# dan11003/tbv_slam_public

Hardware: AMD Instinct MI355X
Metric: radar scan registrations/sec (400x3360 polar) (higher is better)
Workload: dtype u8 filter / f32 search / f64 solve

## Files before the change

tbv_slam_public_amd/csrc/matcher.hip:

```cpp
#include <algorithm>
#include <cfloat>
#include <cmath>
#include <memory>

#include "common.hpp"
#include "fastmath.hpp"

namespace {

#ifdef CFEAR_REG_TIMING
__device__ long long g_reg_t[32];
__device__ unsigned long long g_reg_sum[4];
#define REG_T0() long long _t0 = __builtin_readcyclecounter()
#define REG_TACC(k) do { const long long _t1 = __builtin_readcyclecounter(); \
    if (threadIdx.x == 0 && blockIdx.x == 0) g_reg_t[k] += _t1 - _t0; _t0 = _t1; } while (0)
#else
#define REG_T0()
#define REG_TACC(k)
#endif

constexpr int kMaxScans = kRegMaxScans;
constexpr int kRegDeferred = 1000;

struct MatchCommon {
  cfear_reg_params par;
  double angle_outlier;
  char* scratch;
  size_t scratch_stride;
  size_t job_stride;
  int32_t pairs_cap;
  int32_t dense_fields;
  uint32_t lds_total;
  int32_t cost_only;
  int32_t n_samples;
  int32_t samples_per_axis;
  int32_t only_deferred;
  int32_t take_all;
  int32_t final_launch;
  uint32_t lds_regular;
  cfear_reg_result* results;
  double xy_half, yaw_half;
  const cfear_reg_result* prior;
};

int reg_dense_fields(int cost) { return cost == CFEAR_P2P ? 3 : (cost == CFEAR_P2L ? 5 : 6); }

__host__ __device__ inline size_t match_bytes_global(int pairs_cap) { return ((size_t)pairs_cap * 2 + 255) / 256 * 256; }
size_t reg_scratch_bytes(int pairs_cap) { return match_bytes_global(pairs_cap) + ((size_t)pairs_cap * 52 + 255) / 256 * 256; }

struct Aff2 { double l0, l1, l2, l3, t0, t1; };

__device__ __forceinline__ Aff2 aff_from_xyt(const double* p) {
  double s, c;
  sincos(p[2], &s, &c);
  return Aff2{c, -s, s, c, p[0], p[1]};
}
__device__ __forceinline__ Aff2 aff_mul(const Aff2& a, const Aff2& b) {
  Aff2 r;
  r.l0 = a.l0 * b.l0 + a.l1 * b.l2;
  r.l1 = a.l0 * b.l1 + a.l1 * b.l3;
  r.l2 = a.l2 * b.l0 + a.l3 * b.l2;
  r.l3 = a.l2 * b.l1 + a.l3 * b.l3;
  r.t0 = a.l0 * b.t0 + a.l1 * b.t1 + a.t0;
  r.t1 = a.l2 * b.t0 + a.l3 * b.t1 + a.t1;
  return r;
}
__device__ __forceinline__ Aff2 aff_inv(const Aff2& a) {
  const double det = a.l0 * a.l3 - a.l2 * a.l1;
  const double invdet = 1.0 / det;
  Aff2 r;
  r.l0 = a.l3 * invdet; r.l1 = -a.l1 * invdet; r.l2 = -a.l2 * invdet; r.l3 = a.l0 * invdet;
  r.t0 = -(r.l0 * a.t0 + r.l1 * a.t1);
  r.t1 = -(r.l2 * a.t0 + r.l3 * a.t1);
  return r;
}

__device__ __forceinline__ double similarity(double x, double y) { return 2 * fmin(x, y) / (x + y); }
__device__ __forceinline__ double get_weight(int opt, double N1, double N2, double sim_dir, double plan1, double plan2) {
  switch (opt) {
    case 0: return 1.0;
    case 1: return similarity(N1, N2);
    case 2: return sim_dir;
    case 3: return similarity(plan1, plan2);
    case 4: return similarity(N1, N2) + sim_dir + similarity(plan1, plan2);
  }
  return 1.0;
}

__device__ __forceinline__ void loss_eval(int loss, double a, double w, double s, double& rho0, double& rho1) {
  const double dmin = DBL_MIN;
  switch (loss) {
    case 1: {
      const double b = a * a;
      if (s > b) {
        const double q = rsqrt_newton(s);
        rho0 = 2.0 * a * (s * q) - b; rho1 = fmax(dmin, a * q);
      } else { rho0 = s; rho1 = 1.0; }
      break;
    }
    case 2: {
      const double b = a * a, c = 1.0 / b;
      const double sum = 1.0 + s * c, inv = 1.0 / sum;
      rho0 = b * log(sum); rho1 = fmax(dmin, inv);
      break;
    }
    case 3: {
      const double b = a * a, c = 1.0 / b;
      const double sum = 1.0 + s * c, tmp = sqrt(sum);
      rho0 = 2.0 * b * (tmp - 1.0); rho1 = fmax(dmin, 1.0 / tmp);
      break;
    }
    case 4: {
      const double sum = 1.0 + s, inv = 1.0 / sum;
      const double g0 = log(sum), g1 = fmax(dmin, inv);
      double f0, f1;
      if (g0 > 1.0) { const double r = sqrt(g0); f0 = 2.0 * r - 1.0; f1 = fmax(dmin, 1.0 / r); }
      else { f0 = g0; f1 = 1.0; }
      rho0 = f0; rho1 = f1 * g1;
      break;
    }
    case 5: {
      const double a2 = a * a;
      if (s <= a2) { const double value = 1.0 - s / a2, vs = value * value; rho0 = a2 / 3.0 * (1.0 - vs * value); rho1 = vs; }
      else { rho0 = a2 / 3.0; rho1 = 0.0; }
      break;
    }
    default: rho0 = s; rho1 = 1.0;
  }
  rho0 *= w; rho1 *= w;
}

enum {
  S_X = 0, S_XCOST = 3, S_CUR = 4 , S_SCALE = 13, S_DIAG = 16, S_XNORM = 19, S_GMAX = 20, S_RADIUS = 21,
  S_DEC = 22, S_MINCOST = 23, S_MODEL = 24, S_CAND = 25, S_COS = 28, S_SIN = 29, S_ITCOST = 30, S_ITREL = 31, S_INIT = 32,
  S_LASTREL = 33, S_FINAL = 34, S_INTS = 35 , S_OUTER = 39 , S_COUNT = 48
};
enum { SI_ITER = 0, SI_REUSE = 1, SI_INVALID = 2, SI_PUSHED = 3, SI_USABLE = 4, SI_DONE = 5, SI_ITSUCC = 6, SI_FLAG = 7 };
constexpr int kMaxNW = 16;
constexpr size_t kPartOff = 0;
constexpr size_t kIpartOff = kMaxNW * 10 * 8;
constexpr size_t kStateOff = kIpartOff + 2 * kMaxNW * 4;
constexpr size_t kFixedLds = kStateOff + S_COUNT * 8;
constexpr int kPtrs = 6;

struct MtFit {
  size_t off_smean, off_match, off_region;
  int region;
  int tables_all;
  int dense_cap;
  bool gmatch;
  bool resident;
  bool can;
  bool good;
};
__host__ __device__ inline MtFit mt_fit(size_t lds_total, int last, int sum_pad, int max_pad, int n_src, int fields, bool allow_gmatch) {
  MtFit m;
  size_t off = kFixedLds + (size_t)last * (12 * 8 + kPtrs * 8 + 16) + ((((size_t)last + 1) * 4 + 15) & ~(size_t)15);
  m.off_smean = off; off += (size_t)n_src * 16;
  const size_t n_pairs = (size_t)last * n_src;
  const size_t match_bytes = ((n_pairs + 7) & ~(size_t)7) * 2;
  const size_t need_one = (size_t)kScanGridStartPad * 2 + (size_t)max_pad * 10;
  m.off_match = off;
  m.gmatch = allow_gmatch && ((off + match_bytes + 15) & ~(size_t)15) + need_one > lds_total;
  if (!m.gmatch) off += match_bytes;
  off = (off + 15) & ~(size_t)15;
  m.off_region = off;
  m.tables_all = (int)((size_t)last * kScanGridStartPad * 2 + (size_t)sum_pad * 10);
  const size_t per = (size_t)fields * 8 + 2;
  m.can = sum_pad <= 65535 && n_src < 65536 && off + need_one <= lds_total && off + 4096 <= lds_total;
  m.region = m.can ? (int)(lds_total - off) : 0;
  const size_t dense_all = ((n_pairs + 3) & ~(size_t)3) * per;
// ... 211 lines not shown
  const double i1 = rcp_newton(d1);
  const double t21 = A[7] - l20 * A[3];
  const double l21 = t21 * i1;
  const double d2 = A[8] - l20 * A[6] - l21 * t21;
  if (!(d2 > 0.0)) return false;
  const double i2 = rcp_newton(d2);
  const double z0 = b[0];
  const double z1 = b[1] - l10 * z0;
  const double z2 = b[2] - l20 * z0 - l21 * z1;
  y[2] = z2 * i2;
  y[1] = z1 * i1 - l21 * y[2];
  y[0] = z0 * i0 - l10 * y[1] - l20 * y[2];
  return isfinite(y[0]) && isfinite(y[1]) && isfinite(y[2]);
}

template <bool PIN = false>
__device__ __forceinline__ void sincos_pose(const double a, double* s, double* c) {
  if (fabs(a) <= 1e5) sincos_reduced<PIN>(a, s, c);
  else sincos(a, s, c);
}

struct MtSizes {
  int n_src, sum_pad, max_pad;
  int koff_lane;
  float4 geo_lane;
  bool grids_ok;
};
__device__ __forceinline__ MtSizes mt_sizes(const RegJob& job, const int last) {
  const int lane = threadIdx.x & 63;
  int n = 0;
  float4 g = make_float4(0.f, 0.f, 0.f, 1.f);
  if (lane <= last) n = gload<int>(job.scans[lane].n_cells);
  if (lane < last) g = gload_f4(job.scans[lane].grid_geo);
  const int np = lane < last ? scan_grid_pad(n) : 0;
  const int incl = wave_incl_scan_i32(np);
  MtSizes z;
  z.koff_lane = incl - np;
  z.geo_lane = g;
  z.sum_pad = __builtin_amdgcn_readlane(incl, 63);
  z.max_pad = __builtin_amdgcn_readlane(wave_incl_scan_max_i32(np), 63);
  z.n_src = __builtin_amdgcn_readlane(n, last);
  z.grids_ok = __ballot(lane < last && g.w != 1.f) == 0ull;
  return z;
}

template <int NT>
__device__ void mt_stage_once(const RegJob& job, const MtLds& f, const MtSizes& z) {
  const int tid = threadIdx.x, last = job.n_scans - 1;
  if (tid < last) { f.koff[tid] = z.koff_lane; f.ggeo[tid] = z.geo_lane; }
  if (tid == last) f.koff[last] = z.sum_pad;
  if (tid >= 64 && tid < 64 + last) {
    const int i = tid - 64;
    const Aff2 T = aff_from_xyt(job.poses[i]);
    double* k = f.kf + i * 12;
    k[0] = T.l0; k[1] = T.l1; k[2] = T.l2; k[3] = T.l3; k[4] = T.t0; k[5] = T.t1;
    const ScanView& tv = job.scans[i];
    const void** tp = f.tptr + i * kPtrs;
    tp[0] = tv.mean; tp[1] = tv.normal; tp[2] = tv.nsamples; tp[3] = tv.scale; tp[4] = tv.cov; tp[5] = tv.grid;
  }
  const ScanView& src = job.scans[last];
  for (int s = tid; s < z.n_src; s += NT) f.smean[s] = gload_d2(src.mean + s);
  __syncthreads();
}

template <int NT>
__device__ __forceinline__ void mt_restage(const MtLds& f, int i0, int i1) {
  const int tid = threadIdx.x;
  const int k_lo = f.koff[i0], NP = f.koff[i1] - k_lo;
  constexpr int kCs = kScanGridStartPad / 8;
  constexpr int kKf = NT >= 256 ? 4 : 1, kPer = 2;
  const int xy0 = (i1 - i0) * kCs, ix0 = xy0 + NP / 2;
  uint4* out = (uint4*)f.tables;
  auto dst_of = [&](int i, int j, int rel, int np) {
    return j < kCs ? (i - i0) * kCs + j : (j < kCs + np / 2 ? xy0 + rel / 2 + (j - kCs) : ix0 + rel / 8 + (j - kCs - np / 2));
  };
  for (int ib = i0; ib < i1; ib += kKf) {
    g_u32x4 v[kKf][kPer];
    int dst[kKf][kPer];
    unsigned add[kKf];
#pragma unroll
    for (int q = 0; q < kKf; q++) {
      const int i = ib + q;
#pragma unroll
      for (int h = 0; h < kPer; h++) dst[q][h] = -1;
      add[q] = 0u;
      if (i < i1) {
        const char* blob = (const char*)f.tptr[i * kPtrs + 5];
        const int rel = f.koff[i] - k_lo, np = f.koff[i + 1] - f.koff[i], pieces = kCs + np / 2 + np / 8;
        add[q] = (unsigned)rel * 0x10001u;
#pragma unroll
        for (int h = 0; h < kPer; h++) {
          const int j = tid + h * NT;
          if (j < pieces) {
            v[q][h] = gload<g_u32x4>(blob + (size_t)j * 16);
            dst[q][h] = dst_of(i, j, rel, np);
          }
        }
      }
    }
#pragma unroll
    for (int q = 0; q < kKf; q++)
#pragma unroll
      for (int h = 0; h < kPer; h++)
        if (dst[q][h] >= 0) {
          const unsigned a = dst[q][h] < xy0 ? add[q] : 0u;
          out[dst[q][h]] = make_uint4(v[q][h].x + a, v[q][h].y + a, v[q][h].z + a, v[q][h].w + a);
        }
    for (int i = ib; i < min(ib + kKf, i1); i++) {
      const char* blob = (const char*)f.tptr[i * kPtrs + 5];
      const int rel = f.koff[i] - k_lo, np = f.koff[i + 1] - f.koff[i], pieces = kCs + np / 2 + np / 8;
      for (int j = tid + kPer * NT; j < pieces; j += NT) {
        const g_u32x4 t = gload<g_u32x4>(blob + (size_t)j * 16);
        out[dst_of(i, j, rel, np)] = make_uint4(t.x, t.y, t.z, t.w);
      }
    }
  }
  __syncthreads();
}

template <int NT, bool SLOTS, int COST = -1>
__device__ int mt_associate(const RegJob& job, const MatchCommon& cm, int itr, const MtLds& f, const double* xsrc, double* gl_dense,
                            Dense& dn, int* ipart, int& iphase, bool& staged, const Slots* sl = nullptr) {
  const int tid = threadIdx.x, wave = tid >> 6, lane = tid & 63;
  const int last = job.n_scans - 1;
  const int n_src = gload<int>(job.scans[last].n_cells);
  const int n_pairs = last * n_src;
  const double curr_radius = (itr == 1) ? 2 * cm.par.radius : cm.par.radius;
  const double r2 = curr_radius * curr_radius;
  const float rwin = (float)curr_radius + 1e-3f;
  constexpr int G = kScanGrid;
  constexpr bool GM = NT >= 512;
  auto cost_is = [&](const int v) { return COST >= 0 ? COST == v : cm.par.cost == v; };
  const unsigned magic = n_src ? 0xFFFFFFFFu / (unsigned)n_src : 0u;
  auto split = [&](const int p, int& i, int& s) {
    unsigned q = __umulhi((unsigned)p, magic);
    int r = p - (int)q * n_src;
    if (r >= n_src) { q++; r -= n_src; }
    i = (int)q; s = r;
  };
  REG_T0();
  {
    const int k0 = tid - (NT - 64);
    if (k0 >= 0 && k0 < last) {
      const double* k = f.kf + k0 * 12;
      const Aff2 Ttar{k[0], k[1], k[2], k[3], k[4], k[5]};
      double sn, cs;
      sincos_pose<true>(xsrc[2], &sn, &cs);
      const Aff2 Tst = aff_mul(aff_inv(Ttar), Aff2{cs, -sn, sn, cs, xsrc[0], xsrc[1]});
      double* o = f.kf + k0 * 12 + 6;
      o[0] = Tst.l0; o[1] = Tst.l1; o[2] = Tst.l2; o[3] = Tst.l3; o[4] = Tst.t0; o[5] = Tst.t1;
    }
  }
  int accepted = 0;
  int pend_p = -1, pend_i = 0, pend_best = -1;
  double2 pend_ns = make_double2(0.0, 0.0), pend_nt = make_double2(0.0, 0.0);
  auto gate_pending = [&]() {
    if (pend_p < 0) return;
    int m = -1;
    if (pend_best >= 0) {
      const double* T = f.kf + pend_i * 12 + 6;
      const double nsx = T[0] * pend_ns.x + T[1] * pend_ns.y, nsy = T[2] * pend_ns.x + T[3] * pend_ns.y;
      if (fmax(nsx * pend_nt.x + nsy * pend_nt.y, 0.0) > cm.angle_outlier) m = pend_best;
    }
    if (GM && f.gmatch) gstore<unsigned short>(f.gmatch + pend_p, (unsigned short)m);
    else f.match[pend_p] = (unsigned short)m;
    accepted += (m >= 0);
  };
  for (int i0 = 0; i0 < last;) {
    int i1 = i0, bytes = 0;
    if (f.resident) i1 = last;
    else
      while (i1 < last) {
        const int b = kScanGridStartPad * 2 + (f.koff[i1 + 1] - f.koff[i1]) * 10;
        if (bytes + b > f.region) break;
        bytes += b; i1++;
      }
    if (i1 == i0) return -1;
    if (i0 > 0) __syncthreads();
    if (!(f.resident && staged)) mt_restage<NT>(f, i0, i1);
    else __syncthreads();
    REG_TACC(0);
    const int NP = f.koff[i1] - f.koff[i0];
    const float2* txy = (const float2*)(f.tables + (size_t)(i1 - i0) * kScanGridStartPad);
    const unsigned short* tix = (const unsigned short*)(txy + NP);
    const int lo = i0 * n_src, hi = i1 * n_src;
    int p = lo + ((tid - lo) & (NT - 1));
    for (; p < hi; p += NT) {
      int i, s;
      split(p, i, s);
      const double* T = f.kf + i * 12 + 6;
      const double2 u = f.smean[s];
      const double px = T[0] * u.x + T[1] * u.y + T[4];
      const double py = T[2] * u.x + T[3] * u.y + T[5];
      const float qx = (float)px, qy = (float)py;
      const float4 gg = f.ggeo[i];
      const int cx0 = min(G - 1, max(0, (int)floorf((qx - rwin - gg.x) * gg.z))), cx1 = min(G - 1, max(0, (int)floorf((qx + rwin - gg.x) * gg.z)));
      const int cy0 = min(G - 1, max(0, (int)floorf((qy - rwin - gg.y) * gg.z))), cy1 = min(G - 1, max(0, (int)floorf((qy + rwin - gg.y) * gg.z)));
      unsigned long long bestkey = ~0ull;
      auto visit = [&](const float2 c, const unsigned id) {
        const float dx = __fsub_rn(qx, c.x), dy = __fsub_rn(qy, c.y);
        const float d = __fadd_rn(__fmul_rn(dx, dx), __fmul_rn(dy, dy));
        const unsigned long long key = ((unsigned long long)__float_as_uint(d) << 32) | id;
        bestkey = key < bestkey ? key : bestkey;
      };
      const unsigned short* cs = f.tables + (i - i0) * kScanGridStartPad;
      auto scan_run = [&](int qb, int qe) {
        for (int q = qb; q < qe; q += 2) {
          const int qn = min(q + 1, qe - 1);
          const float2 ca = txy[q], cb = txy[qn];
          const unsigned ia = tix[q], ib = tix[qn];
          visit(ca, ia); visit(cb, ib);
        }
      };
      {
        const int r1 = min(cy0 + 1, cy1), r2c = min(cy0 + 2, cy1);
        const int b0 = cs[cy0 * G + cx0], e0 = cs[cy0 * G + cx1 + 1];
        const int b1 = cs[r1 * G + cx0], e1 = cs[r1 * G + cx1 + 1];
        const int b2 = cs[r2c * G + cx0], e2 = cs[r2c * G + cx1 + 1];
        scan_run(b0, e0);
        if (cy1 > cy0) scan_run(b1, e1);
        if (cy1 > cy0 + 1) scan_run(b2, e2);
        for (int cy = cy0 + 3; cy <= cy1; cy++) scan_run((int)cs[cy * G + cx0], (int)cs[cy * G + cx1 + 1]);
      }
      const int best = bestkey == ~0ull ? -1 : (int)(unsigned)(bestkey & 0xFFFFFFFFu);
      const float bestd = __uint_as_float((unsigned)(bestkey >> 32));
      gate_pending();
      pend_p = p; pend_i = i;
      pend_best = (best >= 0 && (double)bestd < r2) ? best : -1;
      if (pend_best >= 0) {
        pend_ns = gload_d2(job.scans[last].normal + s);
        pend_nt = gload_d2((const double2*)f.tptr[i * kPtrs + 1] + best);
      }
    }
    gate_pending();
    pend_p = -1;
    REG_TACC(1);
    i0 = i1;
  }
  staged = true;
  if (GM && f.gmatch) __threadfence_block();
  int base = 0, total = 0;
  if (!SLOTS) {
    const int incl = wave_incl_scan_i32(accepted);
    base = incl - accepted;
    int* buf = ipart + iphase * kMaxNW;
    if (lane == 63) buf[wave] = incl;
    __syncthreads();
    for (int wv = 0; wv < wave; wv++) base += buf[wv];
    int tt = buf[0];
#pragma unroll
    for (int wv = 1; wv < NT / 64; wv++) tt += buf[wv];
    total = __builtin_amdgcn_readfirstlane(tt);
    iphase ^= 1;
    dn.p = f.dense; dn.cap = f.dense_cap; dn.sidx = (unsigned short*)(f.dense + (size_t)cm.dense_fields * f.dense_cap); dn.smean = f.smean;
    dn.gp = gl_dense; dn.gcap = (size_t)cm.pairs_cap; dn.gsidx = (int*)(gl_dense + (size_t)cm.dense_fields * cm.pairs_cap);
    dn.n = total;
  }
  const size_t cap = SLOTS ? 0 : (size_t)dn.cap, gcap = SLOTS ? 0 : dn.gcap;
  REG_TACC(2);
  {
    struct Gathered {
      int best, i, s, tns, sns;
      double2 nt, tm, ns;
      double tsc, ssc;
      double4 S;
    };
    const ScanView& srcv = job.scans[last];
    auto match_at = [&](int p) -> int {
      if (p >= n_pairs) return 0xFFFF;
      return (GM && f.gmatch) ? (int)gload<unsigned short>(f.gmatch + p) : (int)f.match[p];
    };
    auto gather = [&](int best, int i, int s) {
      Gathered g;
      g.best = best;
      if (g.best == 0xFFFF) g.best = -1;
      g.i = i; g.s = s;
      if (g.best >= 0) {
        const void* const* tp = f.tptr + i * kPtrs;
        g.nt = gload_d2((const double2*)tp[1] + g.best);
        g.tm = gload_d2((const double2*)tp[0] + g.best);
        g.tns = gload<int>((const int32_t*)tp[2] + g.best);
        g.tsc = gload<double>((const double*)tp[3] + g.best);
        g.ns = gload_d2(srcv.normal + s);
        g.sns = gload<int>(srcv.nsamples + s);
        g.ssc = gload<double>(srcv.scale + s);
        if (cost_is(CFEAR_P2D)) g.S = gload_d4((const double4*)tp[4] + g.best);
      }
      return g;
    };
    int c = base, i, s;
    split(tid, i, s);
    int m_next = GM ? match_at(tid + NT) : 0;
    Gathered cur = gather(match_at(tid), i, s);
    for (int p = tid; p < n_pairs; p += NT) {
      split(p + NT, i, s);
      int m_use;
      if (GM) { m_use = m_next; m_next = match_at(p + 2 * NT); }
      else m_use = match_at(p + NT);
      const Gathered nxt = gather(m_use, i, s);
      if (cur.best >= 0) {
        const double* K = f.kf + cur.i * 12;
        const double* T = K + 6;
        const double2 nt = cur.nt, tm = cur.tm, ns = cur.ns;
        const double nsx = T[0] * ns.x + T[1] * ns.y, nsy = T[2] * ns.x + T[3] * ns.y;
        const double direction_similarity = fmax(nsx * nt.x + nsy * nt.y, 0.0);
        const double w = get_weight(cm.par.weight_opt, (double)cur.sns, (double)cur.tns,
                                    direction_similarity, cur.ssc, cur.tsc);
        double e[6];
        e[0] = K[0] * tm.x + K[1] * tm.y + K[4];
        e[1] = K[2] * tm.x + K[3] * tm.y + K[5];
        e[2] = w; e[3] = 0.0; e[4] = 0.0; e[5] = 0.0;
        if (cost_is(CFEAR_P2D)) {
          const double4 S = cur.S;
          const double a00 = K[0] * S.x + K[1] * S.z, a01 = K[0] * S.y + K[1] * S.w;
          const double a10 = K[2] * S.x + K[3] * S.z, a11 = K[2] * S.y + K[3] * S.w;
          const double c00 = (cm.par.regularization + (a00 * K[0] + a01 * K[1])) * cm.par.cov_scale;
          const double c01 = (0.0 + (a00 * K[2] + a01 * K[3])) * cm.par.cov_scale;
          const double c10 = (0.0 + (a10 * K[0] + a11 * K[1])) * cm.par.cov_scale;
          const double c11 = (cm.par.regularization + (a10 * K[2] + a11 * K[3])) * cm.par.cov_scale;
          const double det = c00 * c11 - c10 * c01, invdet = 1.0 / det;
          const double i00 = c11 * invdet, i10 = -c10 * invdet, i11 = c00 * invdet;
          const double l00 = sqrt(i00), l10 = i10 / l00;
          e[3] = l00; e[4] = l10; e[5] = sqrt(i11 - l10 * l10);
        } else if (cost_is(CFEAR_P2L)) {
          e[3] = K[0] * nt.x + K[1] * nt.y;
          e[4] = K[2] * nt.x + K[3] * nt.y;
        }
        if (SLOTS) {
          const int pp = p;
          sl->tmx[pp] = e[0]; sl->tmy[pp] = e[1]; sl->w[pp] = e[2]; sl->a0[pp] = e[3]; sl->a1[pp] = e[4]; sl->a2[pp] = e[5];
          sl->tidx[pp] = cur.best;
        } else {
          const int nf = COST == CFEAR_P2P ? 3 : (COST == CFEAR_P2L ? 5 : (COST == CFEAR_P2D ? 6 : cm.dense_fields));
          if (c < (int)cap) {
            dn.sidx[c] = (unsigned short)cur.s;
#pragma unroll
            for (int k = 0; k < 6; k++) if (k < nf) dn.p[k * cap + c] = e[k];
          } else {
            const size_t g = (size_t)c - cap;
            gstore<int>(dn.gsidx + g, cur.s);
#pragma unroll
            for (int k = 0; k < 6; k++) if (k < nf) gstore<double>(dn.gp + k * gcap + g, e[k]);
          }
        }
        c++;
      } else if (SLOTS) {
        sl->w[p] = -1.0; sl->tidx[p] = -1;
      }
      cur = nxt;
    }
  }
  if (SLOTS) return accepted;
  if (total > (int)cap) __threadfence_block();
  __syncthreads();
  REG_TACC(3);
  return total;
}

template <int NT, int COST, int LOSS>
__device__ void eval_all(const MatchCommon& cm, const Dense& dn, const double x[3], double c, double s, double out[10], double* part) {
  double acc[10];
#pragma unroll
  for (int k = 0; k < 10; k++) acc[k] = 0.0;
  const size_t cap = (size_t)dn.cap, gcap = dn.gcap;
  REG_T0();
  const int n_lds = min(dn.n, (int)cap);
  for (int i = threadIdx.x; i < n_lds; i += NT) {
    double a0 = 0.0, a1 = 0.0, a2 = 0.0;
    const int si = (int)dn.sidx[i];
    const double tmx = dn.p[i], tmy = dn.p[cap + i], w = dn.p[2 * cap + i];
    if (COST != CFEAR_P2P) { a0 = dn.p[3 * cap + i]; a1 = dn.p[4 * cap + i]; }
    if (COST == CFEAR_P2D) a2 = dn.p[5 * cap + i];
    const double2 sm = dn.smean[si];
    eval_slot<COST, LOSS, true>(cm.par, sm.x, sm.y, tmx, tmy, a0, a1, a2, w, x[0], x[1], c, s, acc);
  }
  constexpr int kTailU = COST == CFEAR_P2P ? 4 : 2;
  const int n_tail = dn.n - n_lds;
  for (int g0 = threadIdx.x; g0 < n_tail; g0 += kTailU * NT) {
    int si[kTailU];
    double tmx[kTailU], tmy[kTailU], w[kTailU], a0[kTailU], a1[kTailU], a2[kTailU];
#pragma unroll
    for (int u = 0; u < kTailU; u++) {
      const size_t g = (size_t)min(g0 + u * NT, n_tail - 1);
      si[u] = gload<int>(dn.gsidx + g);
      tmx[u] = gload<double>(dn.gp + g); tmy[u] = gload<double>(dn.gp + gcap + g); w[u] = gload<double>(dn.gp + 2 * gcap + g);
      a0[u] = a1[u] = a2[u] = 0.0;
      if (COST != CFEAR_P2P) { a0[u] = gload<double>(dn.gp + 3 * gcap + g); a1[u] = gload<double>(dn.gp + 4 * gcap + g); }
      if (COST == CFEAR_P2D) a2[u] = gload<double>(dn.gp + 5 * gcap + g);
    }
#pragma unroll
    for (int u = 0; u < kTailU; u++)
      if (g0 + u * NT < n_tail) {
// ... 41 lines not shown
        const double c0 = st[S_CAND], c1 = st[S_CAND + 1], c2 = st[S_CAND + 2];
        x_norm = sqrt_newton(c0 * c0 + c1 * c1 + c2 * c2);
        if (l0) {
          st[S_X] = c0; st[S_X + 1] = c1; st[S_X + 2] = c2;
#pragma unroll
          for (int k = 1; k < 10; k++) st[S_CUR + k - 1] = cnd[k];
        }
        x_cost = cand_cost;
        gradient_max_norm = fmax(fabs(cnd[1]), fmax(fabs(cnd[2]), fabs(cnd[3])));
        it_cost = x_cost; it_success = true;
        const double q = 2.0 * it_rel - 1.0;
        radius = radius * rcp_newton(fmax(1.0 / 3.0, 1.0 - q * q * q));
        radius = fmin(max_radius, radius);
        decrease_factor = 2.0; reuse_diagonal = false;
      } else {
        it_cost = cand_cost; it_success = false;
        radius = radius / decrease_factor; decrease_factor *= 2.0; reuse_diagonal = true;
      }
    }
    mt_lds_order();
  }
  while (proceed) {
    n_pushed++;
    last_rel = it_rel;
    min_iter_cost = fmin(min_iter_cost, it_cost);
    if (iteration >= max_iter || (it_success && gradient_max_norm <= gradient_tolerance) || radius <= min_radius) {
      done = 1;
      break;
    }
    iteration++;
    it_cost = 0.0; it_rel = 0.0; it_success = false;
    const double scale[3] = {st[S_SCALE], st[S_SCALE + 1], st[S_SCALE + 2]};
    double gs[3], Hs[9];
    {
      const double* cur = st + S_CUR - 1;
      gs[0] = cur[1] * scale[0]; gs[1] = cur[2] * scale[1]; gs[2] = cur[3] * scale[2];
      Hs[0] = cur[4] * scale[0] * scale[0]; Hs[1] = cur[5] * scale[0] * scale[1]; Hs[2] = cur[6] * scale[0] * scale[2];
      Hs[3] = Hs[1]; Hs[4] = cur[7] * scale[1] * scale[1]; Hs[5] = cur[8] * scale[1] * scale[2];
      Hs[6] = Hs[2]; Hs[7] = Hs[5]; Hs[8] = cur[9] * scale[2] * scale[2];
    }
    double diagonal[3];
    if (!reuse_diagonal) {
      diagonal[0] = fmin(fmax(Hs[0], min_lm_diagonal), max_lm_diagonal);
      diagonal[1] = fmin(fmax(Hs[4], min_lm_diagonal), max_lm_diagonal);
      diagonal[2] = fmin(fmax(Hs[8], min_lm_diagonal), max_lm_diagonal);
      if (l0) { st[S_DIAG] = diagonal[0]; st[S_DIAG + 1] = diagonal[1]; st[S_DIAG + 2] = diagonal[2]; }
    } else {
      diagonal[0] = st[S_DIAG]; diagonal[1] = st[S_DIAG + 1]; diagonal[2] = st[S_DIAG + 2];
    }
    double A[9];
#pragma unroll
    for (int k = 0; k < 9; k++) A[k] = Hs[k];
    const double inv_radius = rcp_newton(radius);
#pragma unroll
    for (int k = 0; k < 3; k++) A[k * 3 + k] += diagonal[k] * inv_radius;
    double y[3], step[3] = {0, 0, 0};
    const bool solved = chol3_solve(A, gs, y);
    reuse_diagonal = true;
    bool step_is_valid = false;
    model_cost_change = 0.0;
    if (solved) {
      step[0] = -y[0]; step[1] = -y[1]; step[2] = -y[2];
      const double sg = step[0] * gs[0] + step[1] * gs[1] + step[2] * gs[2];
      const double hs0 = Hs[0] * step[0] + Hs[1] * step[1] + Hs[2] * step[2];
      const double hs1 = Hs[3] * step[0] + Hs[4] * step[1] + Hs[5] * step[2];
      const double hs2 = Hs[6] * step[0] + Hs[7] * step[1] + Hs[8] * step[2];
      model_cost_change = -sg - (step[0] * hs0 + step[1] * hs1 + step[2] * hs2) / 2.0;
      step_is_valid = model_cost_change > 0.0;
    }
    if (!step_is_valid) {
      if (++num_consecutive_invalid_steps >= 5) { usable = false; done = 1; break; }
      radius = radius / decrease_factor; decrease_factor *= 2.0; reuse_diagonal = true;
      it_cost = x_cost; it_success = false; it_rel = 0.0;
      mt_lds_order();
      continue;
    }
    num_consecutive_invalid_steps = 0;
    double sn, cs;
    const double c2 = st[S_X + 2] + step[2] * scale[2];
    sincos_pose<true>(c2, &sn, &cs);
    if (l0) {
      st[S_CAND] = st[S_X] + step[0] * scale[0]; st[S_CAND + 1] = st[S_X + 1] + step[1] * scale[1]; st[S_CAND + 2] = c2;
      st[S_COS] = cs; st[S_SIN] = sn;
    }
    break;
  }
  if (l0) {
    st[S_XCOST] = x_cost; st[S_XNORM] = x_norm; st[S_GMAX] = gradient_max_norm; st[S_RADIUS] = radius; st[S_DEC] = decrease_factor;
    st[S_MINCOST] = min_iter_cost; st[S_MODEL] = model_cost_change; st[S_ITCOST] = it_cost; st[S_ITREL] = it_rel;
    st[S_LASTREL] = last_rel;
    if (done) st[S_FINAL] = fmin(st[S_INIT], min_iter_cost);
    si[SI_ITER] = iteration; si[SI_REUSE] = reuse_diagonal; si[SI_INVALID] = num_consecutive_invalid_steps;
    si[SI_PUSHED] = n_pushed; si[SI_USABLE] = usable; si[SI_DONE] = done; si[SI_ITSUCC] = it_success;
  }
}

template <int NT, int COST, int LOSS>
__device__ void lm_solve(const MatchCommon& cm, const Dense& dn, const int max_iter, double* part, double* st, const bool eval_only) {
  const bool w0 = (threadIdx.x >> 6) == 0;
  int* si = (int*)(st + S_INTS);
  double cnd[10];
  {
    const double x[3] = {st[S_OUTER], st[S_OUTER + 1], st[S_OUTER + 2]};
    double s0, c0;
    sincos_pose<true>(x[2], &s0, &c0);
    eval_all<NT, COST, LOSS>(cm, dn, x, c0, s0, cnd, part);
    if (eval_only) {
      if (threadIdx.x == 0) st[S_XCOST] = cnd[0];
      return;
    }
    if (w0) {
      if ((threadIdx.x & 63) == 0) {
        st[S_X] = x[0]; st[S_X + 1] = x[1]; st[S_X + 2] = x[2]; st[S_XCOST] = cnd[0];
#pragma unroll
        for (int k = 1; k < 10; k++) st[S_CUR + k - 1] = cnd[k];
        st[S_SCALE] = 1.0 / (1.0 + sqrt(cnd[4]));
        st[S_SCALE + 1] = 1.0 / (1.0 + sqrt(cnd[7]));
        st[S_SCALE + 2] = 1.0 / (1.0 + sqrt(cnd[9]));
        st[S_DIAG] = 0.0; st[S_DIAG + 1] = 0.0; st[S_DIAG + 2] = 0.0;
        st[S_XNORM] = sqrt_newton(x[0] * x[0] + x[1] * x[1] + x[2] * x[2]);
        st[S_GMAX] = fmax(fabs(cnd[1]), fmax(fabs(cnd[2]), fabs(cnd[3])));
        st[S_RADIUS] = 1e4; st[S_DEC] = 2.0; st[S_MINCOST] = cnd[0]; st[S_MODEL] = 0.0; st[S_ITCOST] = cnd[0]; st[S_ITREL] = 0.0;
        st[S_CAND] = x[0]; st[S_CAND + 1] = x[1]; st[S_CAND + 2] = x[2];
        st[S_INIT] = cnd[0]; st[S_LASTREL] = 0.0; st[S_FINAL] = cnd[0];
        si[SI_ITER] = 0; si[SI_REUSE] = 0; si[SI_INVALID] = 0; si[SI_PUSHED] = 0; si[SI_USABLE] = 1; si[SI_DONE] = 0; si[SI_ITSUCC] = 1;
      }
      mt_lds_order();
      lm_round(st, cnd, false, max_iter);
    }
  }
  for (;;) {
    REG_T0();
    __syncthreads();
    REG_TACC(21);
    if (__builtin_amdgcn_readfirstlane(si[SI_DONE])) break;
    const double cand[3] = {st[S_CAND], st[S_CAND + 1], st[S_CAND + 2]};
    const double cs = st[S_COS], sn = st[S_SIN];
    eval_all<NT, COST, LOSS>(cm, dn, cand, cs, sn, cnd, part);
    REG_TACC(22);
    if (w0) { __builtin_amdgcn_s_setprio(3); lm_round(st, cnd, true, max_iter); __builtin_amdgcn_s_setprio(0); }
    REG_TACC(16);
  }
}

__device__ __forceinline__ void write_capacity(cfear_reg_result* r, const double x[3]) {
  r->pose[0] = x[0]; r->pose[1] = x[1]; r->pose[2] = x[2];
  r->score = 0; r->final_cost = 0; r->num_residuals = 0; r->outer_iters = 0; r->lm_iters = 0;
  r->status = CFEAR_ERR_CAPACITY; r->last_relative_decrease = 0; r->reserved = 0;
}

template <int NW, int COST, int LOSS, bool CO, bool WIDE = false>
__global__ __launch_bounds__(NW * 64, WIDE ? 2 : ((NW == 4 && LOSS < 0) ? 3 : 4)) void matcher_kernel(const RegJob* __restrict__ jobs, const MatchCommon cm) {
  constexpr int NT = NW * 64;
#ifdef CFEAR_REG_TIMING
  if (blockIdx.x == 0 && blockIdx.y == 0 && threadIdx.x == 0 && g_reg_sum[1]) {
    printf("matcher launch: %llu workgroups, mean %llu cycles, longest %llu\n", g_reg_sum[1], g_reg_sum[0] / g_reg_sum[1], g_reg_sum[2]);
    g_reg_sum[0] = g_reg_sum[1] = g_reg_sum[2] = 0;
  }
  const long long t_total0 = __builtin_readcyclecounter();
#endif
  REG_T0();
  extern __shared__ __attribute__((aligned(16))) uint8_t smem[];
  const uint32_t lds_eff = cm.lds_total - (NW >= 8 ? (uint32_t)kPartBigBytes : 0u);
  double* part = NW >= 8 ? (double*)(smem + lds_eff) : (double*)(smem + kPartOff);
  int* ipart = (int*)(smem + kIpartOff);
  double* st = (double*)(smem + kStateOff);
  const RegJob& job = *(const RegJob*)((const char*)jobs + (size_t)blockIdx.x * cm.job_stride);
  const int m_out = CO ? (cm.n_samples > 0 ? cm.n_samples : 1) : 1;
  cfear_reg_result* res = cm.results + (size_t)blockIdx.x * m_out;
  if (cm.only_deferred && res->status != kRegDeferred) return;
  const int last = job.n_scans - 1;
  const MtSizes sz = mt_sizes(job, last);
  const int n_src = sz.n_src, sum_pad = sz.sum_pad, max_pad = sz.max_pad;
  const int n_pairs = last * n_src;
  const size_t scr_idx = (size_t)blockIdx.x * gridDim.y + blockIdx.y;
  char* scr = cm.scratch + scr_idx * cm.scratch_stride;
  const MtFit fit = mt_fit(lds_eff, last, sum_pad, max_pad, n_src, cm.dense_fields, NW >= 8);
  MtLds fl;
  const bool ok = fit.can && sz.grids_ok && n_pairs <= cm.pairs_cap && (cm.take_all || fit.good);
  REG_TACC(8);
  if (ok) {
    mt_carve(smem, fit, last, (unsigned short*)scr, fl);
    mt_stage_once<NT>(job, fl, sz);
  }
  REG_TACC(9);
  if (!ok) {
    if (cm.final_launch) {
      const double larger = (mt_fit((uint32_t)(160 * 1024 - 256 - kPartBigBytes), last, sum_pad, max_pad, n_src, cm.dense_fields, true).can &&
                             sz.grids_ok && n_pairs <= cm.pairs_cap && lds_eff < 160u * 1024u - 256u - (uint32_t)kPartBigBytes) ? 1.0 : 0.0;
      for (int sidx = blockIdx.y * NT + (int)threadIdx.x; sidx < m_out; sidx += (int)gridDim.y * NT) {
        write_capacity(res + sidx, job.poses[last]);
        res[sidx].reserved = larger;
      }
    } else if (threadIdx.x == 0) { res->status = kRegDeferred; res->reserved = 0.0; }
    return;
  }
  double* gl_dense = (double*)(scr + match_bytes_global(cm.pairs_cap));
  Dense dn;
  int iphase = 0;
  bool staged = false;
  const int rpb = COST == CFEAR_P2L ? 1 : 2;
  int git = job.itr ? job.itr : cm.par.itr;
  const bool from_prior = CO && cm.prior;
  if (from_prior) git = cm.prior[blockIdx.x].outer_iters;
  git = __builtin_amdgcn_readfirstlane(git);
  if (threadIdx.x == 0) {
    const double* x0 = from_prior ? cm.prior[blockIdx.x].pose : job.poses[last];
#pragma unroll
    for (int k = 0; k < 3; k++) { st[S_OUTER + k] = x0[k]; st[S_OUTER + 3 + k] = x0[k]; }
    st[S_OUTER + 6] = DBL_MAX;
    st[S_FINAL] = 0.0; st[S_LASTREL] = 0.0;
  }
  __syncthreads();
  bool success = true;
  int itr = 1, lm_iters = 0, num_residuals = 0, solved_residuals = 0, fail_status = CFEAR_OK;
  for (itr = 1;; itr++) {
    int a_itr = itr;
    const int sidx = (int)blockIdx.y + (itr - 1) * (int)gridDim.y;
    if (CO) {
      if (sidx >= m_out) break;
      a_itr = git;
      if (threadIdx.x == 0 && cm.n_samples > 0) {
        const int n = cm.samples_per_axis;
        auto lin = [n](double half, int i) {
          if (n == 1) return -half;
          const double delta = (half - (-half)) / ((double)n - 1.0);
          return i < n - 1 ? -half + delta * (double)i : half;
        };
        st[S_OUTER] = lin(cm.xy_half, (sidx / n) % n) + st[S_OUTER + 3];
        st[S_OUTER + 1] = lin(cm.xy_half, sidx % n) + st[S_OUTER + 4];
        st[S_OUTER + 2] = lin(cm.yaw_half, sidx / (n * n)) + st[S_OUTER + 5];
      }
      __syncthreads();
    } else if (itr > cm.par.max_itr_association || !success) break;
    REG_TACC(12);
    const int n_blocks = mt_associate<NT, false, COST>(job, cm, a_itr, fl, st + S_OUTER, gl_dense, dn, ipart, iphase, staged);
    REG_TACC(10);
    num_residuals = n_blocks * rpb;
    success = num_residuals > 1;
    if (!success && !CO) { fail_status = CFEAR_ERR_TOO_FEW_RESIDUALS; break; }
    if (success) { solved_residuals = num_residuals; lm_solve<NT, COST, LOSS>(cm, dn, cm.par.max_itr_solver, part, st, CO); }
    REG_TACC(11);
    if (CO) {
      if (threadIdx.x == 0) {
        cfear_reg_result* r = res + sidx;
        const double c = success ? st[S_XCOST] : 0.0;
        r->pose[0] = st[S_OUTER]; r->pose[1] = st[S_OUTER + 1]; r->pose[2] = st[S_OUTER + 2];
        r->final_cost = c;
        r->score = success ? c / (double)num_residuals : 0.0;
        r->num_residuals = num_residuals; r->outer_iters = git; r->lm_iters = 0;
        r->status = success ? CFEAR_OK : CFEAR_ERR_TOO_FEW_RESIDUALS;
        r->last_relative_decrease = 0.0; r->reserved = 0.0;
      }
      __syncthreads();
      continue;
    }
    const int* si = (const int*)(st + S_INTS);
    const int n_pushed = __builtin_amdgcn_readfirstlane(si[SI_PUSHED]);
    lm_iters += n_pushed - 1;
    success = __builtin_amdgcn_readfirstlane(si[SI_USABLE]) != 0;
    if (!success) fail_status = CFEAR_ERR_SOLVER;
    const double current_score = st[S_FINAL], prev_score = st[S_OUTER + 6];
    const double rel_improvement = (prev_score - current_score) / prev_score;
    const bool past_min = itr > cm.par.min_itr;
    const bool worse = past_min && (prev_score < current_score);
    const bool small_outer = past_min && !worse && (rel_improvement < cm.par.score_tolerance);
    const bool small_inner = past_min && !worse && !small_outer && (st[S_LASTREL] < cm.par.score_tolerance || n_pushed == 1);
    const bool stop = worse || small_outer || small_inner;
    double xo[3], pp[3];
#pragma unroll
    for (int k = 0; k < 3; k++) {
      const double xk = success ? st[S_X + k] : st[S_OUTER + k];
      pp[k] = st[S_OUTER + 3 + k];
      xo[k] = worse ? pp[k] : xk;
      pp[k] = stop ? pp[k] : xo[k];
    }
    __syncthreads();
    if (threadIdx.x == 0) {
#pragma unroll
      for (int k = 0; k < 3; k++) { st[S_OUTER + k] = xo[k]; st[S_OUTER + 3 + k] = pp[k]; }
      st[S_OUTER + 6] = stop ? prev_score : current_score;
    }
    __syncthreads();
    if (stop) break;
  }
  if (CO) return;
  if (threadIdx.x == 0) {
    res->pose[0] = st[S_OUTER]; res->pose[1] = st[S_OUTER + 1]; res->pose[2] = st[S_OUTER + 2];
    const double final_cost = st[S_FINAL];
    res->final_cost = final_cost;
    res->num_residuals = solved_residuals;
    res->outer_iters = itr;
    res->lm_iters = lm_iters;
    res->last_relative_decrease = st[S_LASTREL];
    res->reserved = mt_fit(cm.lds_regular, last, sum_pad, max_pad, n_src, cm.dense_fields, false).good ? 0.0 : 1.0;
    if (success) { res->score = final_cost / (double)solved_residuals; res->status = CFEAR_OK; }
    else { res->score = 0.0; res->status = fail_status; }
#ifdef CFEAR_REG_TIMING
    {
      const unsigned long long cyc = (unsigned long long)(__builtin_readcyclecounter() - t_total0);
      atomicAdd(&g_reg_sum[0], cyc); atomicAdd(&g_reg_sum[1], 1ull); atomicMax(&g_reg_sum[2], cyc);
    }
    if (blockIdx.x == 0) {
      REG_TACC(13);
      const long long top = g_reg_t[8] + g_reg_t[9] + g_reg_t[10] + g_reg_t[11] + g_reg_t[12] + g_reg_t[13];
      printf("matcher cycles: total %lld = top-level buckets %lld | sizes+carve %lld stage_once %lld association %lld solve %lld outer-loop tests %lld tail %lld\n",
             (long long)(__builtin_readcyclecounter() - t_total0), top, g_reg_t[8], g_reg_t[9], g_reg_t[10], g_reg_t[11], g_reg_t[12], g_reg_t[13]);
      printf("matcher cycles (inside): association: restage %lld nn+gate %lld scan %lld gather %lld | solve: eval %lld reduce %lld round %lld barrier %lld (an LM iteration's evaluation as a whole, eval + reduce + call: %lld) | outer %d lm %d n %d\n",
             g_reg_t[0], g_reg_t[1], g_reg_t[2], g_reg_t[3], g_reg_t[4], g_reg_t[5], g_reg_t[16], g_reg_t[21], g_reg_t[22], itr, lm_iters, num_residuals);
      for (int k = 0; k < 32; k++) g_reg_t[k] = 0;
    }
#endif
  }
}

__global__ __launch_bounds__(256) void assoc_kernel(const RegJob* __restrict__ jobs, const MatchCommon cm, int itr, int32_t* n_blocks_out) {
  constexpr int NT = 256;
  extern __shared__ __attribute__((aligned(16))) uint8_t smem[];
  int* ipart = (int*)(smem + kIpartOff);
  const RegJob& job = jobs[0];
  const int last = job.n_scans - 1;
  const MtSizes sz = mt_sizes(job, last);
  const MtFit fit = mt_fit(cm.lds_total, last, sz.sum_pad, sz.max_pad, sz.n_src, 0, false);
  MtLds fl;
  const bool ok = fit.can && sz.grids_ok && last * sz.n_src <= cm.pairs_cap;
  if (ok) {
    mt_carve(smem, fit, last, nullptr, fl);
    fl.resident = false;
    mt_stage_once<NT>(job, fl, sz);
  }
  if (!ok) {
    if (threadIdx.x == 0) n_blocks_out[0] = -1;
    return;
  }
  const Slots sl = slots_of(cm.scratch, cm.pairs_cap);
  Dense dn;
  int iphase = 0;
  bool staged = false;
  const int mine = mt_associate<NT, true>(job, cm, itr, fl, job.poses[last], nullptr, dn, ipart, iphase, staged, &sl);
  const int incl = wave_incl_scan_i32(mine);
  __syncthreads();
  if ((threadIdx.x & 63) == 63) ipart[threadIdx.x >> 6] = incl;
  __syncthreads();
  if (threadIdx.x == 0) n_blocks_out[0] = ipart[0] + ipart[1] + ipart[2] + ipart[3];
}

struct EvalOut {
  double* raw_r;
  double* raw_j;
  double* rob_r;
  double* neq;
};
__global__ __launch_bounds__(256) void eval_kernel(const RegJob* __restrict__ jobs, const MatchCommon cm, double x0, double x1, double x2,
                                                   EvalOut o) {
  extern __shared__ __attribute__((aligned(16))) uint8_t smem[];
  double* part = (double*)(smem + kPartOff);
  const RegJob& job = jobs[0];
  const int last = job.n_scans - 1;
  const int n_src = *job.scans[last].n_cells;
  const int n_slots = last * n_src;
  const Slots sl = slots_of(cm.scratch, cm.pairs_cap);
  double s, c;
  sincos(x2, &s, &c);
  const double2* smean = job.scans[last].mean;
  double acc[10];
#pragma unroll
  for (int k = 0; k < 10; k++) acc[k] = 0.0;
  for (int slot = threadIdx.x; slot < n_slots; slot += 256) {
    const double w = sl.w[slot];
    if (w < 0.0) continue;
    const double2 sm = smean[slot % n_src];
    const double tmx = sl.tmx[slot], tmy = sl.tmy[slot], a0 = sl.a0[slot], a1 = sl.a1[slot];
    const double a2 = cm.par.cost == CFEAR_P2D ? sl.a2[slot] : 0.0;
    eval_slot_rt<true>(cm.par, sm.x, sm.y, tmx, tmy, a0, a1, a2, w, x0, x1, c, s, acc);
    const double sx = (c * sm.x + (-s) * sm.y) + x0, sy = (s * sm.x + c * sm.y) + x1;
    const double dx = -s * sm.x - c * sm.y, dy = c * sm.x - s * sm.y;
    double r0, r1 = 0.0, j[6] = {0, 0, 0, 0, 0, 0};
    if (cm.par.cost == CFEAR_P2L) {
      const double v0 = sx - tmx, v1 = sy - tmy;
      r0 = v0 * a0 + v1 * a1; j[0] = a0; j[1] = a1; j[2] = dx * a0 + dy * a1;
    } else if (cm.par.cost == CFEAR_P2P) {
      r0 = tmx - sx; r1 = tmy - sy; j[0] = -1.0; j[2] = -dx; j[4] = -1.0; j[5] = -dy;
    } else {
      const double v0 = sx - tmx, v1 = sy - tmy;
      r0 = a0 * v0 + 0.0 * v1; r1 = a1 * v0 + a2 * v1;
      j[0] = a0; j[2] = a0 * dx + 0.0 * dy; j[3] = a1; j[4] = a2; j[5] = a1 * dx + a2 * dy;
    }
    const double sq = (cm.par.cost == CFEAR_P2L) ? r0 * r0 : (r0 * r0 + r1 * r1);
    double rho0, rho1;
    loss_eval(cm.par.loss, cm.par.loss_limit, w, sq, rho0, rho1);
    const double sr = sqrt(rho1);
    if (o.raw_r) { o.raw_r[slot * 2] = r0; o.raw_r[slot * 2 + 1] = r1; }
    if (o.raw_j) for (int k = 0; k < 6; k++) o.raw_j[slot * 6 + k] = j[k];
    if (o.rob_r) { o.rob_r[slot * 2] = r0 * sr; o.rob_r[slot * 2 + 1] = r1 * sr; }
  }
  if (cm.par.cost == CFEAR_P2P) acc[7] = acc[4];
  block_reduce10<4>(acc, part);
  if (threadIdx.x == 0 && o.neq) for (int k = 0; k < 10; k++) o.neq[k] = acc[k];
}

int check_params(cfear_ctx* ctx, const cfear_reg_params* p) {
  if (!p) return cfear_set_error(ctx, CFEAR_ERR_INVALID_ARGUMENT, "null parameters");
  if (p->cost < 0 || p->cost > 2 || p->loss < 0 || p->loss > 5 || p->weight_opt < 0 || p->weight_opt > 4)
    return cfear_set_error(ctx, CFEAR_ERR_INVALID_ARGUMENT, "bad cost/loss/weight option");
  if (p->max_itr_association < 1 || p->max_itr_solver < 0 || !(p->radius > 0))
    return cfear_set_error(ctx, CFEAR_ERR_INVALID_ARGUMENT, "bad iteration limits / radius");
  return CFEAR_OK;
}

typedef void (*MatcherFn)(const RegJob*, MatchCommon);
template <int NW, bool CO>
MatcherFn matcher_fn_nw(int cost, bool huber) {
  switch (cost) {
    case CFEAR_P2P: return huber ? matcher_kernel<NW, CFEAR_P2P, CFEAR_LOSS_HUBER, CO> : matcher_kernel<NW, CFEAR_P2P, -1, CO>;
    case CFEAR_P2L: return huber ? matcher_kernel<NW, CFEAR_P2L, CFEAR_LOSS_HUBER, CO> : matcher_kernel<NW, CFEAR_P2L, -1, CO>;
    default: return huber ? matcher_kernel<NW, CFEAR_P2D, CFEAR_LOSS_HUBER, CO> : matcher_kernel<NW, CFEAR_P2D, -1, CO>;
  }
}
MatcherFn matcher_fn_wide(int cost, bool huber) {
  switch (cost) {
    case CFEAR_P2P: return huber ? matcher_kernel<8, CFEAR_P2P, CFEAR_LOSS_HUBER, false, true> : matcher_kernel<8, CFEAR_P2P, -1, false, true>;
    case CFEAR_P2L: return huber ? matcher_kernel<8, CFEAR_P2L, CFEAR_LOSS_HUBER, false, true> : matcher_kernel<8, CFEAR_P2L, -1, false, true>;
    default: return huber ? matcher_kernel<8, CFEAR_P2D, CFEAR_LOSS_HUBER, false, true> : matcher_kernel<8, CFEAR_P2D, -1, false, true>;
  }
}
MatcherFn matcher_fn(int nw, int cost, bool huber, bool cost_only, bool wide = false) {
  if (cost_only) return nw <= 4 ? matcher_fn_nw<4, true>(cost, huber) : matcher_fn_nw<8, true>(cost, huber);
  if (nw == 8 && wide) return matcher_fn_wide(cost, huber);
  switch (nw) {
    case 2: return matcher_fn_nw<2, false>(cost, huber);
    case 4: return matcher_fn_nw<4, false>(cost, huber);
    case 8: return matcher_fn_nw<8, false>(cost, huber);
    default: return matcher_fn_nw<16, false>(cost, huber);
  }
}

}

size_t cfear_reg_job_bytes() { return sizeof(RegJob); }
int cfear_reg_max_scans() { return kMaxScans; }
void cfear_reg_job_set_itr(void* job, int itr) { ((RegJob*)job)->itr = itr; }
size_t cfear_reg_job_stride(int max_scans) { return reg_job_stride(max_scans); }
size_t cfear_register_scratch_bytes(int pairs_cap) { return reg_scratch_bytes(pairs_cap); }

void cfear_reg_fill_job(void* dst, const ScanView* views, int n_scans, const double* poses_xyt) {
  RegJob* j = (RegJob*)dst;
  j->n_scans = n_scans;
  j->itr = 0;
  for (int i = 0; i < n_scans; i++) {
    j->poses[i][0] = poses_xyt[3 * i]; j->poses[i][1] = poses_xyt[3 * i + 1]; j->poses[i][2] = poses_xyt[3 * i + 2];
    j->scans[i] = views[i];
  }
}

namespace {
constexpr size_t kLdsCu = 160 * 1024;
constexpr size_t kLdsPairs = 20 * 1024;
size_t regular_lds(bool huber) { return huber ? kLdsCu / 4 : (kLdsCu / 3) & ~(size_t)255; }

struct Form { int nw; size_t lds; };
Form first_form(const cfear_ctx* ctx, int n_wgs, bool huber, bool small_pairs, bool big_pass) {
  const int per_cu = std::max(1, (n_wgs + ctx->n_cu - 1) / ctx->n_cu);
  Form f;
// ... 569 lines not shown
```

Baseline: 1.399 million.

## Prefetch first four candidates per grid row with vector loads and merge row scans

Restructures the nearest-neighbour grid search. For each of the first three grid rows it loads an aligned group of four candidate points with float4 loads, then walks the remaining candidates of all three rows in one flattened loop, four at a time. The aim is fewer dependent load round trips and less divergent per-row loop overhead. The cost is predicated extra distance work on out-of-range lanes and more registers; it also adds optional counters and a padding macro that are compiled only for debugging.

Result: no change. 1.408 million, median of 6 (+0.6%).

```diff
diff --git a/tbv_slam_public_amd/csrc/matcher.hip b/tbv_slam_public_amd/csrc/matcher.hip
--- a/tbv_slam_public_amd/csrc/matcher.hip
+++ b/tbv_slam_public_amd/csrc/matcher.hip
@@ -14,9 +14,19 @@
 #define REG_T0() long long _t0 = __builtin_readcyclecounter()
 #define REG_TACC(k) do { const long long _t1 = __builtin_readcyclecounter(); \
     if (threadIdx.x == 0 && blockIdx.x == 0) g_reg_t[k] += _t1 - _t0; _t0 = _t1; } while (0)
+__device__ unsigned long long g_reg_n[4];
+#define REG_NDECL() unsigned _rn[4] = {0u, 0u, 0u, 0u}
+#define REG_NWAVE(k) do { if ((int)(threadIdx.x & 63) == __ffsll((long long)__ballot(1)) - 1) _rn[k]++; } while (0)
+#define REG_NLANE(k, v) do { _rn[k] += (unsigned)(v); } while (0)
+#define REG_NFLUSH() do { if (blockIdx.x == 0 && threadIdx.x < 64) for (int _k = 0; _k < 4; _k++) { unsigned _v = _rn[_k]; \
+    for (int _o = 32; _o; _o >>= 1) _v += __shfl_xor(_v, _o); if (threadIdx.x == 0) g_reg_n[_k] += _v; } } while (0)
 #else
 #define REG_T0()
 #define REG_TACC(k)
+#define REG_NDECL()
+#define REG_NWAVE(k)
+#define REG_NLANE(k, v)
+#define REG_NFLUSH()
 #endif
 
 constexpr int kMaxScans = kRegMaxScans;
@@ -534,6 +544,7 @@
     }
   }
   int accepted = 0;
+  REG_NDECL();
   int pend_p = -1, pend_i = 0, pend_best = -1;
   double2 pend_ns = make_double2(0.0, 0.0), pend_nt = make_double2(0.0, 0.0);
   auto gate_pending = [&]() {
@@ -567,51 +578,108 @@
     const unsigned short* tix = (const unsigned short*)(txy + NP);
     const int lo = i0 * n_src, hi = i1 * n_src;
     int p = lo + ((tid - lo) & (NT - 1));
-    for (; p < hi; p += NT) {
-      int i, s;
-      split(p, i, s);
-      const double* T = f.kf + i * 12 + 6;
-      const double2 u = f.smean[s];
+    struct Win { float qx, qy; int i, s, cx0, cx1, cy0, cy1, b[3], e[3]; };
+    struct Trip { float4 xa[3], xb[3]; unsigned ia[3], ib[3]; };
+    auto window = [&](const int pp) {
+      Win w;
+      split(pp, w.i, w.s);
+      const double* T = f.kf + w.i * 12 + 6;
+      const double2 u = f.smean[w.s];
       const double px = T[0] * u.x + T[1] * u.y + T[4];
       const double py = T[2] * u.x + T[3] * u.y + T[5];
-      const float qx = (float)px, qy = (float)py;
-      const float4 gg = f.ggeo[i];
-      const int cx0 = min(G - 1, max(0, (int)floorf((qx - rwin - gg.x) * gg.z))), cx1 = min(G - 1, max(0, (int)floorf((qx + rwin - gg.x) * gg.z)));
-      const int cy0 = min(G - 1, max(0, (int)floorf((qy - rwin - gg.y) * gg.z))), cy1 = min(G - 1, max(0, (int)floorf((qy + rwin - gg.y) * gg.z)));
+      w.qx = (float)px; w.qy = (float)py;
+      const float4 gg = f.ggeo[w.i];
+      w.cx0 = min(G - 1, max(0, (int)floorf((w.qx - rwin - gg.x) * gg.z))); w.cx1 = min(G - 1, max(0, (int)floorf((w.qx + rwin - gg.x) * gg.z)));
+      w.cy0 = min(G - 1, max(0, (int)floorf((w.qy - rwin - gg.y) * gg.z))); w.cy1 = min(G - 1, max(0, (int)floorf((w.qy + rwin - gg.y) * gg.z)));
+      const unsigned short* cs = f.tables + (w.i - i0) * kScanGridStartPad;
+#pragma unroll
+      for (int r = 0; r < 3; r++) {
+        const int cy = min(w.cy0 + r, w.cy1);
+        const int b = cs[cy * G + w.cx0], e = cs[cy * G + w.cx1 + 1];
+        w.b[r] = b; w.e[r] = w.cy0 + r <= w.cy1 ? e : b;
+      }
+      return w;
+    };
+    auto trip_at = [&](const int b) { return min(b & ~1, NP - 4); };
+    auto first_trip = [&](const Win& w) {
+      Trip t;
+#pragma unroll
+      for (int r = 0; r < 3; r++) {
+        const int q = trip_at(w.b[r]);
+        const float4* x4 = (const float4*)(txy + q);
+        const unsigned* i2 = (const unsigned*)(tix + q);
+        t.xa[r] = x4[0]; t.xb[r] = x4[1]; t.ia[r] = i2[0]; t.ib[r] = i2[1];
+      }
+      return t;
+    };
+    auto finish = [&](const Win& w, const Trip& t) {
+      const float qx = w.qx, qy = w.qy;
       unsigned long long bestkey = ~0ull;
-      auto visit = [&](const float2 c, const unsigned id) {
-        const float dx = __fsub_rn(qx, c.x), dy = __fsub_rn(qy, c.y);
-        const float d = __fadd_rn(__fmul_rn(dx, dx), __fmul_rn(dy, dy));
-        const unsigned long long key = ((unsigned long long)__float_as_uint(d) << 32) | id;
+      auto dist = [&](const float cx, const float cy) {
+        const float dx = __fsub_rn(qx, cx), dy = __fsub_rn(qy, cy);
+        return __fadd_rn(__fmul_rn(dx, dx), __fmul_rn(dy, dy));
+      };
+      auto take = [&](const unsigned dbits, const unsigned id) {
+        const unsigned long long key = ((unsigned long long)dbits << 32) | id;
         bestkey = key < bestkey ? key : bestkey;
       };
-      const unsigned short* cs = f.tables + (i - i0) * kScanGridStartPad;
-      auto scan_run = [&](int qb, int qe) {
+      auto take_if = [&](const bool in, const float cx, const float cy, const unsigned id) {
+        take(in ? __float_as_uint(dist(cx, cy)) : 0xFFFFFFFFu, id);
+      };
+      int s[3], n[3];
+#pragma unroll
+      for (int r = 0; r < 3; r++) {
+        const unsigned len = (unsigned)(w.e[r] - w.b[r]);
+        const int q = trip_at(w.b[r]), off = q - w.b[r];
+        take_if((unsigned)off < len, t.xa[r].x, t.xa[r].y, t.ia[r] & 0xFFFFu);
+        take_if((unsigned)(off + 1) < len, t.xa[r].z, t.xa[r].w, t.ia[r] >> 16);
+        take_if((unsigned)(off + 2) < len, t.xb[r].x, t.xb[r].y, t.ib[r] & 0xFFFFu);
+        take_if((unsigned)(off + 3) < len, t.xb[r].z, t.xb[r].w, t.ib[r] >> 16);
+        s[r] = q + 4; n[r] = max(w.e[r] - s[r], 0);
+        REG_NLANE(3, len);
+      }
+      REG_NWAVE(1);
+      const int n01 = n[0] + n[1], nall = n01 + n[2], d1 = s[1] - n[0], d2 = s[2] - n01;
+      for (int k0 = 0; k0 < nall; k0 += 4) {
+        REG_NWAVE(1);
+        float2 c[4];
+        unsigned id[4];
+#pragma unroll
+        for (int h = 0; h < 4; h++) {
+          const int k = min(k0 + h, nall - 1);
+          const int q = k + (k < n[0] ? s[0] : (k < n01 ? d1 : d2));
+          c[h] = txy[q]; id[h] = tix[q];
+        }
+#pragma unroll
+        for (int h = 0; h < 4; h++) take(__float_as_uint(dist(c[h].x, c[h].y)), id[h]);
+      }
+      const unsigned short* cs = f.tables + (w.i - i0) * kScanGridStartPad;
+      for (int cy = w.cy0 + 3; cy <= w.cy1; cy++) {
+        const int qb = cs[cy * G + w.cx0], qe = cs[cy * G + w.cx1 + 1];
+        REG_NLANE(3, qe - qb);
         for (int q = qb; q < qe; q += 2) {
+          REG_NWAVE(1);
           const int qn = min(q + 1, qe - 1);
           const float2 ca = txy[q], cb = txy[qn];
           const unsigned ia = tix[q], ib = tix[qn];
-          visit(ca, ia); visit(cb, ib);
+          take(__float_as_uint(dist(ca.x, ca.y)), ia); take(__float_as_uint(dist(cb.x, cb.y)), ib);
         }
-      };
-      {
-        const int r1 = min(cy0 + 1, cy1), r2c = min(cy0 + 2, cy1);
-        const int b0 = cs[cy0 * G + cx0], e0 = cs[cy0 * G + cx1 + 1];
-        const int b1 = cs[r1 * G + cx0], e1 = cs[r1 * G + cx1 + 1];
-        const int b2 = cs[r2c * G + cx0], e2 = cs[r2c * G + cx1 + 1];
-        scan_run(b0, e0);
-        if (cy1 > cy0) scan_run(b1, e1);
-        if (cy1 > cy0 + 1) scan_run(b2, e2);
-        for (int cy = cy0 + 3; cy <= cy1; cy++) scan_run((int)cs[cy * G + cx0], (int)cs[cy * G + cx1 + 1]);
       }
+      return bestkey;
+    };
+    for (; p < hi; p += NT) {
+      REG_NWAVE(0); REG_NLANE(2, 1);
+      const Win w = window(p);
+      const Trip t = first_trip(w);
+      const unsigned long long bestkey = finish(w, t);
       const int best = bestkey == ~0ull ? -1 : (int)(unsigned)(bestkey & 0xFFFFFFFFu);
       const float bestd = __uint_as_float((unsigned)(bestkey >> 32));
       gate_pending();
-      pend_p = p; pend_i = i;
+      pend_p = p; pend_i = w.i;
       pend_best = (best >= 0 && (double)bestd < r2) ? best : -1;
       if (pend_best >= 0) {
-        pend_ns = gload_d2(job.scans[last].normal + s);
-        pend_nt = gload_d2((const double2*)f.tptr[i * kPtrs + 1] + best);
+        pend_ns = gload_d2(job.scans[last].normal + w.s);
+        pend_nt = gload_d2((const double2*)f.tptr[w.i * kPtrs + 1] + best);
       }
     }
     gate_pending();
@@ -620,6 +688,7 @@
     i0 = i1;
   }
   staged = true;
+  REG_NFLUSH();
   if (GM && f.gmatch) __threadfence_block();
   int base = 0, total = 0;
   if (!SLOTS) {
@@ -967,6 +1036,9 @@
 template <int NW, int COST, int LOSS, bool CO, bool WIDE = false>
 __global__ __launch_bounds__(NW * 64, WIDE ? 2 : ((NW == 4 && LOSS < 0) ? 3 : 4)) void matcher_kernel(const RegJob* __restrict__ jobs, const MatchCommon cm) {
   constexpr int NT = NW * 64;
+#ifdef MT_HEAD_PAD
+  asm volatile(".rept %0\n s_nop 0\n .endr" :: "n"(MT_HEAD_PAD * 4));
+#endif
 #ifdef CFEAR_REG_TIMING
   if (blockIdx.x == 0 && blockIdx.y == 0 && threadIdx.x == 0 && g_reg_sum[1]) {
     printf("matcher launch: %llu workgroups, mean %llu cycles, longest %llu\n", g_reg_sum[1], g_reg_sum[0] / g_reg_sum[1], g_reg_sum[2]);
@@ -1123,7 +1195,11 @@
              (long long)(__builtin_readcyclecounter() - t_total0), top, g_reg_t[8], g_reg_t[9], g_reg_t[10], g_reg_t[11], g_reg_t[12], g_reg_t[13]);
       printf("matcher cycles (inside): association: restage %lld nn+gate %lld scan %lld gather %lld | solve: eval %lld reduce %lld round %lld barrier %lld (an LM iteration's evaluation as a whole, eval + reduce + call: %lld) | outer %d lm %d n %d\n",
              g_reg_t[0], g_reg_t[1], g_reg_t[2], g_reg_t[3], g_reg_t[4], g_reg_t[5], g_reg_t[16], g_reg_t[21], g_reg_t[22], itr, lm_iters, num_residuals);
+      printf("matcher search (wavefront 0): pair steps %llu round trips %llu (%.2f per step) | pairs %llu records %llu (%.2f per pair)\n",
+             g_reg_n[0], g_reg_n[1], (double)g_reg_n[1] / (double)max(g_reg_n[0], 1ull), g_reg_n[2], g_reg_n[3],
+             (double)g_reg_n[3] / (double)max(g_reg_n[2], 1ull));
       for (int k = 0; k < 32; k++) g_reg_t[k] = 0;
+      for (int k = 0; k < 4; k++) g_reg_n[k] = 0;
     }
 #endif
   }
```
